# weilonghu/KGC-GCN

Hardware: AMD Instinct MI355X
Metric: aggregated_edges_per_sec (higher is better)
Workload: dtype f32 (dense step as six bf16-split MFMA products, f32 accumulation: f32-faithful); 1 GPU; wn18rr-shape synthetic graph (N=40943, R=11, E=86835), 2-layer M-GCN encoder 100->200->200, full-graph forward, eval mode; n_ranks_seen=1

## Files before the change

kgc-gcn_amd/csrc/layer_fused2.hip:

```cpp
#include <hip/hip_runtime.h>

#include <cstdlib>
#include <type_traits>

#include "fused_common.h"

namespace {

constexpr int T2 = 1024;

struct Args2 : LayerArgs {
  int32_t nch, nkb_last, kbm, G;
  float bn_eps;
#ifdef MGCN_DIAG
  unsigned long long *stamps;
  int32_t ablate;
#endif
};
#ifdef MGCN_DIAG
#define MGCN_ABLATE(bit) (p.ablate & (bit))
#define MGCN_STAMP(role, idx)                                                                                      \
  do {                                                                                                             \
    if (p.stamps && lane == 0 && (idx) < 128) p.stamps[(int64_t(blockIdx.x) * 2 + (role)) * 128 + (idx)] = __builtin_readcyclecounter(); \
  } while (0)
#else
#define MGCN_ABLATE(bit) 0
#define MGCN_STAMP(role, idx) do {} while (0)
#endif

constexpr int EPI_FLOATS = 2 * 208;
constexpr int REL_LDS_MAX_BYTES = 32 * 1024;

template <int NT, int NRT, bool RELLDS, bool HUBS>
__global__ __launch_bounds__(T2, 4) void layer_fused2_kernel(Args2 p) {
  constexpr int BM = NRT * 16;
  constexpr int PIECE = 16 * BM * 16;
  constexpr int BUF = 3 * PIECE;
  constexpr int RPG = BM / 16;
  constexpr int UB = 4;
  constexpr int CH = 32 / UB * UB;
  extern __shared__ __attribute__((aligned(16))) unsigned char lds2[];
  float *epi = reinterpret_cast<float *>(lds2 + 2 * BUF);
  float *rel_lds = epi + EPI_FLOATS;

  const int bid = int(blockIdx.x), nblk = int(gridDim.x);
  const int tid = threadIdx.x;
  const int wave = __builtin_amdgcn_readfirstlane(tid >> 6), lane = tid & 63;
  const int nrows = p.node1 - p.node0;
  const int ntiles = (nrows + BM - 1) / BM;
  const int my_tiles = (ntiles - bid + nblk - 1) / nblk;
  const int nch = p.nch;

#ifdef MGCN_DIAG
  if (p.stamps && lane == 0 && (wave == 0 || wave == 8)) {
    p.stamps[(int64_t(blockIdx.x) * 2 + (wave ? 1 : 0)) * 128 + 120] = __builtin_readcyclecounter();
    p.stamps[(int64_t(blockIdx.x) * 2 + (wave ? 1 : 0)) * 128 + 121] = __builtin_amdgcn_s_memrealtime();
  }
#endif
  auto stage_barrier = [] () __attribute__((always_inline)) {
    asm volatile("s_waitcnt lgkmcnt(0)\n\ts_barrier" ::: "memory");
  };
  if (wave >= 8) {
    __builtin_amdgcn_s_setprio(3);
    const int gtid = tid - 512;
    const int grp = gtid >> 5, lig = gtid & 31;
    const int glane0 = lane & 32;
    const int g_lo = grp * RPG, g_hi = g_lo + RPG;
    const int qcol = lig >> 1, frot = (qcol >> 1) & 7;
    const int wbase = qcol * BM * 16 + (lig & 1) * 8;
    const uint32_t ldx32 = uint32_t(p.ldx), d32 = uint32_t(p.d);

    auto write_row = [&](unsigned char *img, int row, float4 v, bool ok) __attribute__((always_inline)) {
      uint32_t h[2], m[2], l[2];
      split3p(ok ? v.x : 0.f, ok ? v.y : 0.f, h[0], m[0], l[0]);
      split3p(ok ? v.z : 0.f, ok ? v.w : 0.f, h[1], m[1], l[1]);
      unsigned char *dst = img + wbase + ((row & ~15) + (((row & 15) + frot) & 15)) * 16;
      *reinterpret_cast<uint2 *>(dst) = make_uint2(h[0], h[1]);
      *reinterpret_cast<uint2 *>(dst + PIECE) = make_uint2(m[0], m[1]);
      *reinterpret_cast<uint2 *>(dst + 2 * PIECE) = make_uint2(l[0], l[1]);
    };
    auto rp_of = [&](int it_, int mode_) {
      return rp_load(p.rowptr + int64_t(mode_) * (p.n + 1), p.node0 + (bid + it_ * nblk) * BM, BM, p.node1, lig);
    };
    auto rp_get = [&](const RowPtrs &r, int idx) {
      const int from = glane0 + (idx & 31);
      const int va = __shfl(r.a, from), vb = __shfl(r.b, from), vc = __shfl(r.c, from);
      return idx < 32 ? va : (idx < 64 ? vb : vc);
    };
    struct Part { int lo, hi, rp; };
    auto partition = [&](const RowPtrs &r) {
      const int base = __shfl(r.a, glane0);
      const int tot = rp_get(r, BM) - base;
      const int c = 2 > (tot >> 8) + 1 ? 2 : (tot >> 8) + 1;
      const int ptot = tot + c * BM;
      const int thr_lo = (grp * ptot) >> 4, thr_hi = ((grp + 1) * ptot) >> 4;
      int lo = 0, hi = 0;
      const int vals[3] = {r.a, r.b, r.c};
#pragma unroll
      for (int k = 0; k < 3; ++k) {
        const int i = lig + 32 * k;
        const int pw = (vals[k] - base) + c * i;
        const unsigned long long blo = __ballot(i < BM && pw < thr_lo), bhi = __ballot(i < BM && pw < thr_hi);
        lo += __popc(uint32_t(blo >> glane0));
        hi += __popc(uint32_t(bhi >> glane0));
      }
      Part q;
      q.lo = lo; q.hi = hi;
      const int idx = lo + (lig < hi - lo ? lig : hi - lo);
      const int from = glane0 + (idx & 31);
      const int va = __shfl(r.a, from), vb = __shfl(r.b, from), vc = __shfl(r.c, from);
      q.rp = idx < 32 ? va : (idx < 64 ? vb : vc);
      return q;
    };
    auto rec_chunk = [&](int cbeg, int end) {
      int4 r = make_int4(0, 0, 0, 0);
      if (end > cbeg) r = p.rec[(cbeg + lig < end) ? cbeg + lig : end - 1];
      return r;
    };
    Part cur = partition(rp_of(0, 0));
    int4 currec = rec_chunk(__shfl(cur.rp, glane0), __shfl(cur.rp, glane0 + (cur.hi - cur.lo)));
    int stage = 0;
    for (int it = 0; it < my_tiles; ++it) {
      const int r0 = p.node0 + (bid + it * nblk) * BM;
      for (int mi = 0; mi < 3; ++mi) {
        const int mode = mi == 0 ? 2 : mi - 1;
        if (mode < 2) {
          const int myrp = cur.rp, e_lo = cur.lo, e_hi = cur.hi, e_n = cur.hi - cur.lo;
          const int4 firstrec = currec;
          const int ee_sub_mode = p.ee_sub[mode];
          const bool has_next = mode == 0 || it + 1 < my_tiles;
          RowPtrs nrp = {0, 0, 0};
          if (has_next) nrp = rp_of(mode == 0 ? it : it + 1, mode == 0 ? 1 : 0);
          Part nxt = {0, 0, 0};
          bool next_recs_issued = false;
          int4 nrec = make_int4(0, 0, 0, 0);
          auto prefetch_next = [&]() __attribute__((always_inline)) {
            if (has_next) {
              nxt = partition(nrp);
              nrec = rec_chunk(__shfl(nxt.rp, glane0), __shfl(nxt.rp, glane0 + (nxt.hi - nxt.lo)));
            }
          };
          int2 myhub = make_int2(-1, 0);
          {
            const int node = r0 + e_lo + lig;
            if (HUBS && p.hubinfo && lig < e_n && node < p.node1) myhub = p.hubinfo[int64_t(mode) * p.n + node];
          }
          const int beg = __shfl(myrp, glane0), end = MGCN_ABLATE(1) ? beg : __shfl(myrp, glane0 + e_n);
          for (int chunk = 0; chunk < nch; ++chunk, ++stage) {
            if (wave == 8) MGCN_STAMP(1, 2 * stage);
            unsigned char *img = lds2 + (stage & 1) * BUF;
            const int coff_ = chunk * 128 + lig * 4;
            const bool col_ok = coff_ < p.d;
            const int coff = col_ok ? coff_ : 0;
            const float *xb = p.x + coff, *relb = (RELLDS ? rel_lds : p.rel) + coff, *eeb = p.ee + coff;
            int4 myrec = firstrec;
            int row = e_lo, nb = __shfl(myrp, glane0 + 1);
            float4 sum = make_float4(0.f, 0.f, 0.f, 0.f);
            auto flush = [&]() __attribute__((always_inline)) {
              if (HUBS && p.hubinfo) {
                const int first = __shfl(myhub.x, glane0 + (row - e_lo)), cnt = __shfl(myhub.y, glane0 + (row - e_lo));
                if (cnt > 0) {
                  const float4 ps = *reinterpret_cast<const float4 *>(p.partial + int64_t(first - p.chunk0) * p.d + coff);
                  sum = make_float4(sum.x + ps.x, sum.y + ps.y, sum.z + ps.z, sum.w + ps.w);
                }
              }
              write_row(img, row, sum, col_ok);
              sum = make_float4(0.f, 0.f, 0.f, 0.f);
              ++row;
            };
            int cbase = beg;
#ifdef MGCN_DIAG
            int bstamp = 64;
            if (wave == 8 && stage == 1) { MGCN_STAMP(1, 63); }
#endif
            for (int s = beg; s < end; s += UB) {
              if (s >= cbase + CH) {
                cbase += CH;
                myrec = rec_chunk(cbase, end);
              }
              int rsrc[UB], rtyp[UB], rnrm[UB];
#pragma unroll
              for (int u = 0; u < UB; ++u) {
                const int from = glane0 + (((s + u < end) ? s + u : end - 1) - cbase);
                rsrc[u] = __shfl(myrec.x, from);
                rtyp[u] = __shfl(myrec.y, from);
                rnrm[u] = __shfl(myrec.z, from);
              }
              float4 xv[UB], rv[UB], ev[UB];
#pragma unroll
              for (int u = 0; u < UB; ++u) {
                if (MGCN_ABLATE(16)) rsrc[u] = 0;
                xv[u] = *reinterpret_cast<const float4 *>(xb + uint64_t(uint32_t(rsrc[u])) * ldx32);
                if (!RELLDS) rv[u] = *reinterpret_cast<const float4 *>(relb + uint64_t(uint32_t(rtyp[u])) * d32);
                const uint32_t erow = MGCN_ABLATE(16) ? 0u : uint32_t(((s + u < end) ? s + u : end - 1) - ee_sub_mode);
                ev[u] = *reinterpret_cast<const float4 *>(eeb + uint64_t(erow) * d32);
              }
#ifdef MGCN_DIAG
              if (wave == 8 && stage == 1 && bstamp < 126) { MGCN_STAMP(1, bstamp); ++bstamp; }
#endif
              if (!next_recs_issued) {
                next_recs_issued = true;
                prefetch_next();
              }
#ifdef MGCN_DIAG
              if (wave == 8 && stage == 1 && bstamp < 126) {
                asm volatile("s_waitcnt vmcnt(0)" ::: "memory");
                MGCN_STAMP(1, bstamp); ++bstamp;
              }
#endif
#pragma unroll
              for (int u = 0; u < UB; ++u) {
                if (s + u < end) {
                  while (s + u >= nb) {
                    flush();
                    nb = __shfl(myrp, glane0 + (row - e_lo) + 1);
                  }
                  const float4 rr = RELLDS ? *reinterpret_cast<const float4 *>(relb + uint32_t(rtyp[u]) * d32) : rv[u];
                  const float4 m = f4mul(f4mul(xv[u], rr), ev[u]);
                  const float wgt = __int_as_float(rnrm[u]);
                  sum = make_float4(sum.x + m.x * wgt, sum.y + m.y * wgt, sum.z + m.z * wgt, sum.w + m.w * wgt);
                }
              }
            }
            if (!next_recs_issued) {
              next_recs_issued = true;
              prefetch_next();
            }
#ifdef MGCN_DIAG
            if (wave == 8 && stage == 1 && bstamp < 126) { MGCN_STAMP(1, bstamp); ++bstamp; }
#endif
            while (row < e_hi) flush();
            if (wave == 8) MGCN_STAMP(1, 2 * stage + 1);
            stage_barrier();
          }
          cur = nxt;
          currec = nrec;
        } else {
          for (int chunk = 0; chunk < nch; ++chunk, ++stage) {
            if (wave == 8) MGCN_STAMP(1, 2 * stage);
            unsigned char *img = lds2 + (stage & 1) * BUF;
            const int coff_ = chunk * 128 + lig * 4;
            const bool col_ok = coff_ < p.d;
            const int coff = col_ok ? coff_ : 0;
            const float4 lr = *reinterpret_cast<const float4 *>(p.loop_rel + coff);
            const float4 le = *reinterpret_cast<const float4 *>(p.loop_edge + coff);
            float4 xs[RPG];
#pragma unroll
            for (int i = 0; i < RPG; ++i) {
              const int node = (r0 + g_lo + i < p.node1) ? r0 + g_lo + i : p.node1 - 1;
              xs[i] = *reinterpret_cast<const float4 *>(p.x + int64_t(node) * p.ldx + coff);
            }
#pragma unroll
            for (int i = 0; i < RPG; ++i) write_row(img, g_lo + i, f4mul(f4mul(xs[i], lr), le), col_ok);
            if (wave == 8) MGCN_STAMP(1, 2 * stage + 1);
            stage_barrier();
          }
        }
      }
    }
    if (p.rel_out) rel_projection(p, wave, 8, 8, lane, bid, nblk);
#ifdef MGCN_DIAG
    if (p.stamps && lane == 0 && wave == 8) {
      p.stamps[(int64_t(blockIdx.x) * 2 + 1) * 128 + 122] = __builtin_readcyclecounter();
      p.stamps[(int64_t(blockIdx.x) * 2 + 1) * 128 + 123] = __builtin_amdgcn_s_memrealtime();
    }
#endif
  } else {
    auto multiply = [&](auto Hc) __attribute__((always_inline)) {
    constexpr int H = decltype(Hc)::value;
    constexpr int QALL = NT / 4, R = NT % 4;
    constexpr int QA = (QALL + 1) / 2;
    constexpr int Q = H == 0 ? QA : QALL - QA;
    constexpr int QF = Q > 0 ? Q : 1;
    constexpr int NX = H == 1 ? R * NRT : 0;
    constexpr int XE = (NX + 3) / 4;
    constexpr int XF = XE > 0 ? XE : 1;
    constexpr int XW = (R == 1) ? 1 : XF;
    const int w = wave & 3;
    const int r = lane & 15, gq = lane >> 4;
    const int ct0 = w * QALL + (H == 0 ? 0 : QA);
    int xct[XF], xrt[XF];
    bool xok[XF];
#pragma unroll
    for (int j = 0; j < XF; ++j) {
      const int e = 4 * j + w;
      xok[j] = XE > 0 && e < NX;
      xct[j] = xok[j] ? 4 * QALL + e / NRT : 0;
      xrt[j] = xok[j] ? e % NRT : -1;
    }
    const int G = p.G;
    auto wload = [&](u32x4 (&wq)[QF][3], u32x4 (&wx)[XW][3], int g) {
      if (MGCN_ABLATE(8)) g = 0;
      if (MGCN_ABLATE(64) && g != 0) return;
      const u32x4 *base = p.wp + (int64_t(g) * NT) * 3 * 64 + lane;
#pragma unroll
      for (int t = 0; t < Q; ++t) {
#pragma unroll
        for (int pc = 0; pc < 3; ++pc) wq[t][pc] = base[((ct0 + t) * 3 + pc) * 64];
      }
      if (XE > 0) {
#pragma unroll
        for (int j = 0; j < XW; ++j) {
#pragma unroll
          for (int pc = 0; pc < 3; ++pc) wx[j][pc] = base[(xct[j] * 3 + pc) * 64];
        }
      }
    };
    u32x4 wq0[QF][3], wx0[XW][3], wq1[QF][3], wx1[XW][3], wq2[QF][3], wx2[XW][3];

    f32x4 acc[NRT][QF], accx[XF];
    auto zero_acc = [&]() {
#pragma unroll
      for (int rt = 0; rt < NRT; ++rt) {
#pragma unroll
        for (int t = 0; t < QF; ++t) acc[rt][t] = f32x4{0.f, 0.f, 0.f, 0.f};
      }
#pragma unroll
      for (int j = 0; j < XF; ++j) accx[j] = f32x4{0.f, 0.f, 0.f, 0.f};
    };
    auto store_unit = [&](f32x4 a, int prow, int col, const float4 &sc, const float4 &sh) {
      if (prow < nrows) {
        const float4 v = make_float4(tanh_fast(fmaf(a[0], sc.x, sh.x)), tanh_fast(fmaf(a[1], sc.y, sh.y)),
                                     tanh_fast(fmaf(a[2], sc.z, sh.z)), tanh_fast(fmaf(a[3], sc.w, sh.w)));
        *reinterpret_cast<float4 *>(p.out + int64_t(prow) * p.ldo + col) = v;
      }
    };
    auto epilogue = [&](int tile) {
      const int prow0 = tile * BM + r;
      auto column_tile = [&](int ct, auto &&body) {
        const int col = ct * 16 + 4 * gq;
        if (col < p.o) body(col, *reinterpret_cast<const float4 *>(epi + col), *reinterpret_cast<const float4 *>(epi + 208 + col));
      };
#pragma unroll
      for (int t = 0; t < Q; ++t) {
        column_tile(ct0 + t, [&](int col, const float4 &sc, const float4 &sh) {
#pragma unroll
          for (int rt = 0; rt < NRT; ++rt) store_unit(acc[rt][t], prow0 + rt * 16, col, sc, sh);
        });
      }
      if (XE > 0) {
#pragma unroll
        for (int j = 0; j < XF; ++j) {
          if (xok[j])
            column_tile(xct[j], [&](int col, const float4 &sc, const float4 &sh) { store_unit(accx[j], prow0 + xrt[j] * 16, col, sc, sh); });
        }
      }
    };

    auto rotated = [&](int kb_, int) { return kb_; };
    int kb = 0, chunk = 0, stage = 0;
    bool barrier_done = false;
    int nkb_ = 0, nchunk = 0, nmode = 0;
    auto advance_next = [&]() {
      const int n = (nchunk == nch - 1) ? p.nkb_last : 4;
      if (++nkb_ == n) {
        nkb_ = 0;
        if (++nchunk == nch) {
          nchunk = 0;
          nmode = nmode == 2 ? 0 : nmode + 1;
        }
      }
    };
    auto gindex = [&]() {
      const int mode_ = nmode == 0 ? 2 : nmode - 1;
      return mode_ * p.kbm + 4 * nchunk + rotated(nkb_, nchunk);
    };
    wload(wq0, wx0, gindex());
    advance_next();
    if (H == 0) {
      const int t8 = (wave & 3) * 64 + lane;
      if (t8 < 208) epilogue_table_entry(p, p.bn_eps, epi, 208, t8);
    }
    if (RELLDS) copy_rel_table(p, rel_lds, wave, lane, 8);
    auto kblock = [&](u32x4 (&wq)[QF][3], u32x4 (&wx)[XW][3], u32x4 (&nq)[QF][3], u32x4 (&nx)[XW][3]) {
      wload(nq, nx, gindex());
      advance_next();
      const int nkb_c = (chunk == nch - 1) ? p.nkb_last : 4;
      if (kb == 0) {
        if (!barrier_done) stage_barrier();
        barrier_done = false;
        if (wave == 0) MGCN_STAMP(0, 2 * stage);
      }
      const int qc = 4 * rotated(kb, chunk) + gq;
      const unsigned char *ap = lds2 + (stage & 1) * BUF + (qc * BM + ((r + ((qc >> 1) & 7)) & 15)) * 16;
      constexpr int WP[6] = {0, 2, 1, 0, 1, 0}, AP[6] = {2, 0, 1, 1, 0, 0};
#pragma unroll
      for (int rt = 0; rt < NRT; ++rt) {
        if (Q > 0 && !MGCN_ABLATE(2)) {
          bf16x8 a[3];
#pragma unroll
          for (int pc = 0; pc < 3; ++pc)
            a[pc] = __builtin_bit_cast(bf16x8, MGCN_ABLATE(32) ? wq[0][pc] : *reinterpret_cast<const u32x4 *>(ap + pc * PIECE + rt * 256));
#pragma unroll
          for (int pr = 0; pr < 6; ++pr) {
#pragma unroll
            for (int t = 0; t < Q; ++t)
              acc[rt][t] = __builtin_amdgcn_mfma_f32_16x16x32_bf16(__builtin_bit_cast(bf16x8, wq[t][WP[pr]]), a[AP[pr]],
                                                                   acc[rt][t], 0, 0, 0);
          }
        }
      }
      if (XE > 0) {
#pragma unroll
        for (int j = 0; j < XF; ++j) {
          if (xok[j]) {
            bf16x8 a[3];
#pragma unroll
            for (int pc = 0; pc < 3; ++pc)
              a[pc] = __builtin_bit_cast(bf16x8, MGCN_ABLATE(32) ? wx[0][pc] : *reinterpret_cast<const u32x4 *>(ap + pc * PIECE + xrt[j] * 256));
#pragma unroll
            for (int pr = 0; pr < 6; ++pr)
              accx[j] = __builtin_amdgcn_mfma_f32_16x16x32_bf16(__builtin_bit_cast(bf16x8, wx[XW == 1 ? 0 : j][WP[pr]]),
                                                                a[AP[pr]], accx[j], 0, 0, 0);
          }
        }
      }
      if (++kb == nkb_c) {
        if (wave == 0) MGCN_STAMP(0, 2 * stage + 1);
        if (stage < 8) MGCN_STAMP(0, 32 + 8 * stage + wave);
        kb = 0;
        ++stage;
        if (++chunk == nch) chunk = 0;
      }
    };
    for (int it = 0; it < my_tiles; ++it) {
      zero_acc();
      for (int g0 = 0; g0 < G; g0 += 3) {
        kblock(wq0, wx0, wq1, wx1);
        kblock(wq1, wx1, wq2, wx2);
        kblock(wq2, wx2, wq0, wx0);
      }
      if (it + 1 < my_tiles) {
        stage_barrier();
        barrier_done = true;
      }
      if (wave == 0) MGCN_STAMP(0, 100 + 2 * it);
      if (!MGCN_ABLATE(4)) epilogue(bid + it * nblk);
      if (wave == 0) MGCN_STAMP(0, 101 + 2 * it);
    }
#ifdef MGCN_DIAG
    if (p.stamps && lane == 0 && wave == 0) {
      p.stamps[int64_t(blockIdx.x) * 2 * 128 + 122] = __builtin_readcyclecounter();
      p.stamps[int64_t(blockIdx.x) * 2 * 128 + 123] = __builtin_amdgcn_s_memrealtime();
    }
#endif
    };
    if (wave < 4) multiply(std::integral_constant<int, 0>{});
    else multiply(std::integral_constant<int, 1>{});
  }
}

template <int NT, int NRT, bool RELLDS, bool HUBS>
int launch2(const Args2 &p, int grid, hipStream_t st) {
  constexpr size_t lds_bytes = size_t(2) * 3 * 16 * (NRT * 16) * 16 + EPI_FLOATS * 4 + (RELLDS ? REL_LDS_MAX_BYTES : 0);
  if (hipFuncSetAttribute(reinterpret_cast<const void *>(&layer_fused2_kernel<NT, NRT, RELLDS, HUBS>),
                          hipFuncAttributeMaxDynamicSharedMemorySize, int(lds_bytes)) != hipSuccess)
    return mgcn::fail(MGCN_ELAUNCH, "layer_fused2: cannot reserve %zu bytes of LDS", lds_bytes);
  hipLaunchKernelGGL((layer_fused2_kernel<NT, NRT, RELLDS, HUBS>), dim3(unsigned(grid)), dim3(T2), lds_bytes, st, p);
  MGCN_CHECK_LAUNCH("layer_fused2_kernel");
  return MGCN_OK;
}

int pick_nt2(int o) { return o <= 32 ? 2 : o <= 64 ? 4 : o <= 128 ? 8 : 13; }

struct Shape2 {
  int nch, nkb_last, kbm, G;
};
Shape2 shape2(int d) {
  Shape2 s;
  s.nch = (d + 127) / 128;
  const int wlast = d - 128 * (s.nch - 1);
  s.nkb_last = (wlast + 31) / 32;
  s.kbm = 4 * (s.nch - 1) + s.nkb_last;
  s.G = 3 * s.kbm;
  return s;
}

#ifdef MGCN_DIAG
unsigned long long *diag_stamps() {
  static unsigned long long *buf = nullptr;
  if (!buf && getenv("MGCN_FUSED_STAMPS")) {
    if (hipMalloc(&buf, 1024 * 2 * 128 * 8) != hipSuccess) buf = nullptr;
    else (void)hipMemset(buf, 0, 1024 * 2 * 128 * 8);
  }
  return buf;
}
#endif

}

#ifdef MGCN_DIAG
extern "C" int mgcn_diag_read_stamps(unsigned long long *host_out) {
  unsigned long long *b = diag_stamps();
  if (!b) return 1;
  return hipMemcpy(host_out, b, 1024 * 2 * 128 * 8, hipMemcpyDeviceToHost) == hipSuccess ? 0 : 2;
}
#endif

namespace mgcn {

bool fused2_takes(int32_t dim_in, int32_t dim_out) {
  return dim_in > 0 && dim_in % 4 == 0 && dim_in <= 1024 && dim_out > 0 && dim_out % 4 == 0 && dim_out <= 208;
}

size_t fused2_packed_bytes(int32_t dim_in, int32_t dim_out) { return pack_modes_bytes(dim_in, pick_nt2(dim_out)); }

int fused2_pack(int32_t dim_in, int32_t dim_out, const float *w_dev, void *wp_dev, void *stream) {
  const int kbm = pack_modes_kbm(dim_in);
  return pack_launch(wp_dev, 3 * kbm, pick_nt2(dim_out), ModeWeights{w_dev, dim_in, dim_out, kbm}, stream);
}

int fused2_launch(const FusedLaunch &a) {
  const int32_t dim_in = a.dim_in, dim_out = a.dim_out;
  const Shape2 s = shape2(dim_in);
  Args2 p = {};
  fill_layer_args(p, a);
  p.nch = s.nch; p.nkb_last = s.nkb_last; p.kbm = s.kbm; p.G = s.G;
  p.bn_eps = a.bn_eps;
#ifdef MGCN_DIAG
  if (const char *ab = getenv("MGCN_FUSED_ABLATE")) p.ablate = atoi(ab);
  p.stamps = diag_stamps();
#endif
  const int cus = cu_count();
  const int64_t nrows = a.node_end - a.node_begin;
  auto grid_for = [&](int rt) { const int64_t t = (nrows + rt * 16 - 1) / (rt * 16); return int(t < cus ? (t > 0 ? t : 1) : cus); };
  auto makespan = [&](int bm) { return ((nrows + bm - 1) / bm + cus - 1) / cus * bm; };
  int nrt = makespan(64) < makespan(80) ? 4 : 5;
#ifdef MGCN_DIAG
  if (const char *e = getenv("MGCN_FUSED_NRT")) nrt = atoi(e) == 4 ? 4 : 5;
#endif
  const int grid = grid_for(nrt);
  hipStream_t st = static_cast<hipStream_t>(a.stream);
  const bool rel_lds = a.rel && size_t(a.num_rel_rows - 1) * dim_in * 4 <= size_t(REL_LDS_MAX_BYTES);
  const bool hubs = a.hubinfo != nullptr;
  switch (pick_nt2(dim_out)) {
    case 2: return launch2<2, 5, false, true>(p, grid_for(5), st);
    case 4: return launch2<4, 5, false, true>(p, grid_for(5), st);
    case 8: return launch2<8, 5, false, true>(p, grid_for(5), st);
    default:
      if (nrt == 4) {
        if (rel_lds) return hubs ? launch2<13, 4, true, true>(p, grid, st) : launch2<13, 4, true, false>(p, grid, st);
        return hubs ? launch2<13, 4, false, true>(p, grid, st) : launch2<13, 4, false, false>(p, grid, st);
      }
      if (rel_lds) return hubs ? launch2<13, 5, true, true>(p, grid, st) : launch2<13, 5, true, false>(p, grid, st);
      return hubs ? launch2<13, 5, false, true>(p, grid, st) : launch2<13, 5, false, false>(p, grid, st);
  }
}

}
```

Measured before the change: 2.783 billion edges/s.

## Use buffer stores in epilogue and prefetch next tile weights before it

The epilogue now writes output through a buffer resource descriptor with hardware range checking instead of branchy per-row guarded global stores. Out-of-range lanes are redirected to an out-of-bounds offset so the stores become unconditional. Weight prefetch is moved so the second weight group is loaded before the epilogue runs, overlapping that load with the epilogue stores for the next tile. A stride limit check is added because the offsets are now 32-bit.

```diff
diff --git a/kgc-gcn_amd/csrc/layer_fused2.hip b/kgc-gcn_amd/csrc/layer_fused2.hip
--- a/kgc-gcn_amd/csrc/layer_fused2.hip
+++ b/kgc-gcn_amd/csrc/layer_fused2.hip
@@ -289,6 +289,7 @@
       xrt[j] = xok[j] ? e % NRT : -1;
     }
     const int G = p.G;
+    const uint32_t ldo32 = uint32_t(p.ldo);
     auto wload = [&](u32x4 (&wq)[QF][3], u32x4 (&wx)[XW][3], int g) {
       if (MGCN_ABLATE(8)) g = 0;
       if (MGCN_ABLATE(64) && g != 0) return;
@@ -318,31 +319,34 @@
 #pragma unroll
       for (int j = 0; j < XF; ++j) accx[j] = f32x4{0.f, 0.f, 0.f, 0.f};
     };
-    auto store_unit = [&](f32x4 a, int prow, int col, const float4 &sc, const float4 &sh) {
-      if (prow < nrows) {
-        const float4 v = make_float4(tanh_fast(fmaf(a[0], sc.x, sh.x)), tanh_fast(fmaf(a[1], sc.y, sh.y)),
-                                     tanh_fast(fmaf(a[2], sc.z, sh.z)), tanh_fast(fmaf(a[3], sc.w, sh.w)));
-        *reinterpret_cast<float4 *>(p.out + int64_t(prow) * p.ldo + col) = v;
-      }
+    auto store_unit = [&](f32x4 a, __amdgpu_buffer_rsrc_t out_tile, uint32_t voff, int rt, const float4 &sc, const float4 &sh) {
+      const f32x4 v = {tanh_fast(fmaf(a[0], sc.x, sh.x)), tanh_fast(fmaf(a[1], sc.y, sh.y)),
+                       tanh_fast(fmaf(a[2], sc.z, sh.z)), tanh_fast(fmaf(a[3], sc.w, sh.w))};
+      __builtin_amdgcn_raw_buffer_store_b128(__builtin_bit_cast(u32x4, v), out_tile, int(voff), int(uint32_t(rt) * 64u * ldo32), 0);
+      __builtin_amdgcn_sched_barrier(0);
     };
     auto epilogue = [&](int tile) {
-      const int prow0 = tile * BM + r;
+      const int left = nrows - tile * BM;
+      const uint32_t bytes = uint32_t(left < BM ? left : BM) * ldo32 * 4u;
+      const __amdgpu_buffer_rsrc_t out_tile = __builtin_amdgcn_make_buffer_rsrc(p.out + int64_t(tile) * BM * p.ldo, 0, int(bytes), 0x00020000);
       auto column_tile = [&](int ct, auto &&body) {
         const int col = ct * 16 + 4 * gq;
-        if (col < p.o) body(col, *reinterpret_cast<const float4 *>(epi + col), *reinterpret_cast<const float4 *>(epi + 208 + col));
+        body((uint32_t(r) * ldo32 + uint32_t(col)) * 4u, col < p.o, *reinterpret_cast<const float4 *>(epi + col),
+             *reinterpret_cast<const float4 *>(epi + 208 + col));
       };
 #pragma unroll
       for (int t = 0; t < Q; ++t) {
-        column_tile(ct0 + t, [&](int col, const float4 &sc, const float4 &sh) {
-#pragma unroll
-          for (int rt = 0; rt < NRT; ++rt) store_unit(acc[rt][t], prow0 + rt * 16, col, sc, sh);
+        column_tile(ct0 + t, [&](uint32_t off, bool ok, const float4 &sc, const float4 &sh) {
+#pragma unroll
+          for (int rt = 0; rt < NRT; ++rt) store_unit(acc[rt][t], out_tile, ok && rt * 16 + r < left ? off : bytes, rt, sc, sh);
         });
       }
       if (XE > 0) {
 #pragma unroll
         for (int j = 0; j < XF; ++j) {
-          if (xok[j])
-            column_tile(xct[j], [&](int col, const float4 &sc, const float4 &sh) { store_unit(accx[j], prow0 + xrt[j] * 16, col, sc, sh); });
+          column_tile(xct[j], [&](uint32_t off, bool ok, const float4 &sc, const float4 &sh) {
+            store_unit(accx[j], out_tile, ok && xok[j] && xrt[j] * 16 + r < left ? off : bytes, xok[j] ? xrt[j] : 0, sc, sh);
+          });
         }
       }
     };
@@ -367,14 +371,18 @@
     };
     wload(wq0, wx0, gindex());
     advance_next();
+    wload(wq1, wx1, gindex());
+    advance_next();
     if (H == 0) {
       const int t8 = (wave & 3) * 64 + lane;
       if (t8 < 208) epilogue_table_entry(p, p.bn_eps, epi, 208, t8);
     }
     if (RELLDS) copy_rel_table(p, rel_lds, wave, lane, 8);
-    auto kblock = [&](u32x4 (&wq)[QF][3], u32x4 (&wx)[XW][3], u32x4 (&nq)[QF][3], u32x4 (&nx)[XW][3]) {
-      wload(nq, nx, gindex());
-      advance_next();
+    auto kblock = [&](auto Firstc, u32x4 (&wq)[QF][3], u32x4 (&wx)[XW][3], u32x4 (&nq)[QF][3], u32x4 (&nx)[XW][3]) {
+      if (!decltype(Firstc)::value) {
+        wload(nq, nx, gindex());
+        advance_next();
+      }
       const int nkb_c = (chunk == nch - 1) ? p.nkb_last : 4;
       if (kb == 0) {
         if (!barrier_done) stage_barrier();
@@ -423,20 +431,31 @@
         if (++chunk == nch) chunk = 0;
       }
     };
-    for (int it = 0; it < my_tiles; ++it) {
+    constexpr std::false_type Later{};
+    auto tile_kblocks = [&]() __attribute__((always_inline)) {
       zero_acc();
-      for (int g0 = 0; g0 < G; g0 += 3) {
-        kblock(wq0, wx0, wq1, wx1);
-        kblock(wq1, wx1, wq2, wx2);
-        kblock(wq2, wx2, wq0, wx0);
-      }
+      kblock(std::true_type{}, wq0, wx0, wq1, wx1);
+      kblock(Later, wq1, wx1, wq2, wx2);
+      kblock(Later, wq2, wx2, wq0, wx0);
+      for (int g0 = 3; g0 < G; g0 += 3) {
+        kblock(Later, wq0, wx0, wq1, wx1);
+        kblock(Later, wq1, wx1, wq2, wx2);
+        kblock(Later, wq2, wx2, wq0, wx0);
+      }
+    };
+    tile_kblocks();
+    for (int it = 0;; ++it) {
       if (it + 1 < my_tiles) {
         stage_barrier();
         barrier_done = true;
       }
+      wload(wq1, wx1, gindex());
+      advance_next();
       if (wave == 0) MGCN_STAMP(0, 100 + 2 * it);
       if (!MGCN_ABLATE(4)) epilogue(bid + it * nblk);
       if (wave == 0) MGCN_STAMP(0, 101 + 2 * it);
+      if (it + 1 == my_tiles) break;
+      tile_kblocks();
     }
 #ifdef MGCN_DIAG
     if (p.stamps && lane == 0 && wave == 0) {
@@ -512,6 +531,7 @@
 
 int fused2_launch(const FusedLaunch &a) {
   const int32_t dim_in = a.dim_in, dim_out = a.dim_out;
+  if (a.ldo >= (int64_t(1) << 22)) return mgcn::fail(MGCN_EUNSUPPORTED, "layer_fused2: output row stride %lld too large", (long long)a.ldo);
   const Shape2 s = shape2(dim_in);
   Args2 p = {};
   fill_layer_args(p, a);
```

New measurement: 2.801 billion edges/s (median of 6 runs). No clear change (+0.7%).
